# wangjunchi/LLMSeg

Measured on AMD Instinct MI355X. Metric: images/sec (1024x1024, 64-tok prompt) model_forward fwd+bwd, higher is better.
Workload: dtype bf16; 1 GPU; BASELINE.json configs[2]: synthetic 1024x1024 + random-init LLaVA-7B(Llama-7B+CLIP-L/14)/SAM-ViT-H, batch_size=2 per GPU, fwd+bwd train step (CE + align + IoP losses, LoRA r=8 dropout 0.05 on q/v + trainable embed/lm_head/text_fcs/lisa_*, frozen towers, fp32 gradient arena, AdamW step every 10 micro-steps inside the timed region, micro-step replayed from a hipGraph), 256 candidate masks, 64-token ; global_batch=2, parallelism=dp1, graph=True, valid=True

## Files before the change

llmseg_amd/csrc/capi.cpp:

```cpp
#include <hip/hip_runtime.h>
#include <stdarg.h>
#include <stdio.h>
#include <stdlib.h>
#include <algorithm>
#include <array>
#include <map>
#include <mutex>
#include <string>
#include <vector>
#include "llmseg_hip.h"

static thread_local char g_err[512] = "";

void llmseg_set_error(const char* fmt, ...) {
  va_list ap;
  va_start(ap, fmt);
  vsnprintf(g_err, sizeof(g_err), fmt, ap);
  va_end(ap);
}

extern "C" const char* llmseg_last_error(void) { return g_err; }

#include <atomic>
static std::atomic<long> g_launches{0};
// ... 73 lines not shown
    float t = 0;
    (void)hipEventElapsedTime(&t, r.a, r.b);
    ms += t;
    fl += r.flops;
    auto& c = by_class[((r.tag[3] % 10000) / 1000) * 2 + (r.tag[3] & 1)];
    c[0] += t; c[1] += r.flops; c[2] += 1;
    {
      const long S = r.tag[3] / 10000;
      auto& sp = split_by_class[((r.tag[3] % 10000) / 1000) * 2 + (r.tag[3] & 1)];
      if (S > 1) { sp[0] += 1; sp[1] += S; }
    }
    c[3] += 2.0 * ((double)r.tag[0] * r.tag[2] + (double)r.tag[1] * r.tag[2] + (double)r.tag[0] * r.tag[1]);
    auto& e = by_shape[{r.tag[0], r.tag[1], r.tag[2], r.tag[3]}];
    e[0] += t; e[1] += r.flops; e[2] += 1;
    g_pool.push_back(r);
  }
  if (getenv("LLMSEG_PROF_TABLE")) {
    std::vector<std::pair<double, std::array<long, 4>>> order;
    for (auto& kv : by_shape) order.push_back({-kv.second[0], kv.first});
    std::sort(order.begin(), order.end());
    fprintf(stderr, "%8s %8s %8s %6s %8s %10s %9s %6s\n", "M", "N", "K", "var", "calls", "total_ms", "TFLOP/s", "%time");
    const size_t top = (size_t)std::max(40, atoi(getenv("LLMSEG_PROF_TABLE")));
    for (size_t i = 0; i < order.size() && i < top; ++i) {
      auto& e = by_shape[order[i].second];
      fprintf(stderr, "%8ld %8ld %8ld %6ld %8.0f %10.2f %9.1f %6.1f\n", order[i].second[0], order[i].second[1], order[i].second[2], order[i].second[3],
              e[2], e[0], e[1] / (e[0] * 1e-3) / 1e12, 100.0 * e[0] / ms);
    }
  }
  if (total_ms) *total_ms = ms;
  if (total_flops) *total_flops = fl;
  if (launches) *launches = (int64_t)g_recs.size();
  long dom = -1;
  for (auto& kv : by_class) if (dom < 0 || kv.second[0] > by_class[dom][0]) dom = kv.first;
  static const char* names[] = {"gemm_bf16_tn_kernel<*, ...> (register staging, 128x128)", "?", "gemm_bf16_tn_glds_kernel<*, 2, 1>", "gemm_skinny_kernel<M>", "?", "?", "gemm_bf16_tn_t160_kernel (K-sliced)", "gemm_bf16_tn_pp2_kernel<*, false>",
                                "gemm_bf16_tn_pp_kernel<*, false, 4>", "gemm_bf16_tn_pp_kernel<*, false, 2>"};
  if (dom >= 0) {
    const long v = dom / 2;
    std::string nm = (v >= 0 && v < 10) ? names[v] : "?";
    const size_t star = nm.find('*');
    if (star != std::string::npos) nm.replace(star, 1, (dom & 1) ? "true" : "false");
    snprintf(g_dom_name, sizeof(g_dom_name), "%s", nm.c_str());
  } else g_dom_name[0] = 0;
  if (dom_ms) *dom_ms = dom >= 0 ? by_class[dom][0] : 0;
  if (dom_flops) *dom_flops = dom >= 0 ? by_class[dom][1] : 0;
  if (dom_launches) *dom_launches = dom >= 0 ? (int64_t)by_class[dom][2] : 0;
  g_dom_bytes = dom >= 0 ? by_class[dom][3] : 0;
  if (dom >= 0) {
    const auto& sp = split_by_class[dom];
    g_dom_info[0] = (int64_t)by_class[dom][2]; g_dom_info[1] = sp[0]; g_dom_info[2] = sp[1]; g_dom_info[3] = (int64_t)by_class[dom][2] + sp[0];
  } else g_dom_info[0] = g_dom_info[1] = g_dom_info[2] = g_dom_info[3] = 0;
  g_recs.clear();
  return LLMSEG_OK;
}
```

llmseg_amd/csrc/gemm.hip:

```cpp
#include <algorithm>
#include <cstdlib>
#include "common.h"
#include "llmseg_hip.h"

namespace {

constexpr int BN = 128, BK = 64, NT = 256;
constexpr int GROUP_M = 8;

struct GemmP {
  const bf16_t* A; const bf16_t* W; void* C;
  const bf16_t* bias; const bf16_t* gamma; const bf16_t* res;
  int M, N, K;
  long lda, ldw, ldc, ldr, sA, sW, sC, sA2, sW2, sC2;
  int batch1;
  float alpha;
  int act;
  int tiles_m, tiles_n;
  int c_vec, r_vec, b_vec;
  const bf16_t* A2; const bf16_t* W2; long lda2, ldw2;
  int group_m;
  int skew;
  int kt_total;
  int accum;
// ... 890 lines not shown
  const int n = n0 + wn * 64 + c * 4;
  const int mw = m0 + wm * 80;
  float* cbase = reinterpret_cast<float*>(p.C) + b1 * p.sC;
#pragma unroll
  for (int i = 0; i < 3; ++i) {
    const int nh = i < 2 ? 2 : 1;
#pragma unroll
    for (int h = 0; h < nh; ++h)
#pragma unroll
      for (int nb = 0; nb < 4; ++nb) {
        const int row = h * 16 + r15, chunk = nb * 4 + q4;
        *reinterpret_cast<float4*>(slab + row * 64 + ((chunk ^ (row & 15)) << 2)) =
            make_float4(acc[nb][2 * i + h][0], acc[nb][2 * i + h][1], acc[nb][2 * i + h][2], acc[nb][2 * i + h][3]);
      }
#pragma unroll
    for (int it = 0; it < 4 * nh; ++it) {
      const int row = it * 4 + rsub;
      const float4 a4 = *reinterpret_cast<const float4*>(slab + row * 64 + ((c ^ (row & 15)) << 2));
      const int m = mw + i * 32 + row;
      if (m >= p.M || n >= p.N) continue;
      *reinterpret_cast<float4*>(cbase + (long)m * p.ldc + n) =
          make_float4(fmaf(a4.x, p.alpha, 0.f), fmaf(a4.y, p.alpha, 0.f), fmaf(a4.z, p.alpha, 0.f), fmaf(a4.w, p.alpha, 0.f));
    }
  }
}
#undef T160_BL
#undef T160_ISSUE_A0
#undef T160_ISSUE_A1
#undef T160_ISSUE_W
#undef T160_VM_TILE
#undef T160_READ_A
#undef T160_MMA

template <int MT, int AT, bool SK = false>
__global__ __launch_bounds__(256) void gemm_skinny_kernel(GemmP p, int out_f32) {
  constexpr int KS = MT >= 4 ? 1 : 2;
  constexpr int STEP = KS * 512;
  constexpr int ADV = SK ? 4 * STEP : STEP;
  constexpr int XB = AT == 2 ? MT : 1;
  const int lane = threadIdx.x & 63, wave = threadIdx.x >> 6;
  const int n0 = SK ? blockIdx.x * 4 : (blockIdx.x * 4 + wave) * 4;
  if (n0 >= p.N) return;
  const bf16_t* wr[4];
#pragma unroll
  for (int r = 0; r < 4; ++r) wr[r] = p.W + (long)min(n0 + r, p.N - 1) * p.ldw;
  float acc[4][MT];
#pragma unroll
  for (int r = 0; r < 4; ++r)
#pragma unroll
    for (int m = 0; m < MT; ++m) acc[r][m] = 0.f;
  const int K = p.K;
  auto loadw = [&](uint4 (&w)[KS][4], int k) {
#pragma unroll
    for (int t = 0; t < KS; ++t)
#pragma unroll
      for (int r = 0; r < 4; ++r) w[t][r] = *reinterpret_cast<const uint4*>(wr[r] + min(k + t * 512, K - 8));
  };
  auto loadx = [&](uint4 (&xa)[KS][MT], uint4 (&xb)[KS][XB], int k) {
#pragma unroll
    for (int t = 0; t < KS; ++t) {
      const int kk = k + t * 512, kc = min(kk, K - 8);
      const bool ok = kk < K;
#pragma unroll
      for (int m = 0; m < MT; ++m) {
        const bf16_t* ar = p.A + (long)min(m, p.M - 1) * p.lda;
        const uint4 v = *reinterpret_cast<const uint4*>(ar + kc);
// ... 239 lines not shown
    const int c = threadIdx.x + 256 * i;
    if (c < nch) {
      const int n = c * 8;
      const float* sp = slab + m * p.N + n;
      float4 a0 = *reinterpret_cast<const float4*>(sp), a1 = *reinterpret_cast<const float4*>(sp + 4);
      for (int s2 = 1; s2 < S; ++s2) {
        const float4 b0 = *reinterpret_cast<const float4*>(sp + s2 * slab_sz), b1 = *reinterpret_cast<const float4*>(sp + s2 * slab_sz + 4);
        a0.x += b0.x; a0.y += b0.y; a0.z += b0.z; a0.w += b0.w;
        a1.x += b1.x; a1.y += b1.y; a1.z += b1.z; a1.w += b1.w;
      }
      const float v[8] = {a0.x * p.alpha, a0.y * p.alpha, a0.z * p.alpha, a0.w * p.alpha, a1.x * p.alpha, a1.y * p.alpha, a1.z * p.alpha, a1.w * p.alpha};
      const uint4 g = pack8(v);
      *reinterpret_cast<uint4*>(reinterpret_cast<bf16_t*>(p.C) + m * p.ldc + n) = g;
      float of[8], df[8];
      unpack8(*reinterpret_cast<const uint4*>(O + m * ldo + n), of);
      unpack8(g, df);
      float part = 0.f;
#pragma unroll
      for (int e = 0; e < 8; ++e) part = fmaf(of[e], df[e], part);
#pragma unroll
      for (int mm = 8; mm >= 1; mm >>= 1) part += __shfl_xor(part, mm, 64);
      if ((c & 15) == 0) delta[(b * heads + (c >> 4)) * T + q] = part;
    }
  }
}

enum GemmKernel {
  K_REG = 0,
  K_GLDS = 2,
  K_AUTO = 5,
  K_PP256 = 8,
  K_PP128 = 9,
  K_T160 = 10,
};
inline bool is_pp(GemmKernel k) { return k == K_PP256 || k == K_PP128 || k == K_T160; }
inline int pp_rows(GemmKernel k) { return k == K_PP256 ? 256 : k == K_T160 ? T160_BM : 128; }
inline GemmKernel kernel_of_knob(int v) { return v == K_REG || v == K_GLDS || is_pp((GemmKernel)v) ? (GemmKernel)v : K_AUTO; }

template <bool OUT_F32, bool EXT, int FX = FX_NONE>
void launch_pp(GemmKernel k, const GemmP& p, dim3 grid, hipStream_t s) {
  if (k == K_PP256) LL_LAUNCH_KERNEL((gemm_bf16_tn_pp_kernel<OUT_F32, EXT, FX>), grid, dim3(NTB), 0, s, p);
  else LL_LAUNCH_KERNEL((gemm_bf16_tn_pp2_kernel<OUT_F32, EXT, FX>), grid, dim3(NTB), 0, s, p);
}

enum TailKind {
  TAIL_NORM,
  TAIL_NB,
  TAIL_DL,
  TAIL_FX,
};
struct GemmTail { TailKind kind; const llmseg_gemm_args* req; bool done; };

}

void llmseg_prof_begin(hipStream_t s);
void llmseg_prof_end(hipStream_t s, double flops);
void llmseg_prof_tag(long a, long b, long c, long d);

static int g_gemm_variant = K_AUTO, g_gemm_skew = 13, g_gemm_split = 0;
static const bool g_gemm_t160 = getenv("LLMSEG_GEMM_NO_T160") == nullptr;
static const int g_gemm_rsplit = getenv("LLMSEG_GEMM_NO_RSPLIT") ? 0 : 1;
static int num_cus() {
  static int n = [] { int dev = 0, v = 0; (void)hipGetDevice(&dev); (void)hipDeviceGetAttribute(&v, hipDeviceAttributeMultiprocessorCount, dev); return v > 0 ? v : 256; }();
  return n;
}
extern "C" int llmseg_gemm_set_variant(int v) {
  g_gemm_variant = v & 15;
  if ((v >> 4) & 15) g_gemm_skew = ((v >> 4) & 15) - 1;
  g_gemm_split = (v >> 8) & 31;
  return LLMSEG_OK;
}

namespace {
struct GemmPlan { GemmKernel kernel; int split; double us; };
constexpr double T160_KT_US = 1.13;
inline double pp_cost(long M, long N, int nt, int bm, int S, long ncu, bool f32out) {
  const long tiles = ((M + bm - 1) / bm) * ((N + 255) / 256);
  const long rounds = (tiles * S + ncu - 1) / ncu;
  const int q = (nt + S - 1) / S;
  const double it = bm == 256 ? 1.7 : bm == 160 ? T160_KT_US : 1.0, fix = (bm == 256 ? 7.0 : 4.5) + ((S > 1 || f32out) ? 1.0 : 0.0);
  double eff_rounds = (double)rounds;
  if (S == 1) {
    const long full = tiles / ncu, rem = tiles - full * ncu;
    eff_rounds = (double)full + (rem ? 0.5 + 0.5 * (double)rem / (double)ncu : 0.0);
  }
  double us = eff_rounds * (q * it + fix);
  if (S > 1) us += 2.5 + ((double)(S + 1) * M * N * 4.0) / 4.0e6;
  return us;
}
inline double glds_cost(long M, long N, int nt, long ncu) {
  const long tiles = ((M + 127) / 128) * ((N + 127) / 128);
  const long full = tiles / (4 * ncu), rem = tiles - full * 4 * ncu;
  double us = (double)full * (nt * 2.4 + 4.0);
  if (rem > 0) { const double w = (double)((rem + ncu - 1) / ncu); us += nt * std::max(1.3, 0.6 * w) + 4.0; }
  return us;
}
inline bool split_ok(int nt, int S) {
  if (S <= 1) return S == 1;
  const int q = (nt + S - 1) / S;
  return q >= 2 && nt - (S - 1) * q >= 2;
}
}

static int gemm_dispatch(const llmseg_gemm_args* a, void* stream, GemmTail* tail);

extern "C" int llmseg_norm(const void* x, const void* w, const void* b, void* y, int64_t rows, int64_t cols, int64_t ldx, int64_t ldy, float eps, int rms,
                           const int32_t* row_map, void* stream);

extern "C" int llmseg_rope(void* x, const float* cos, const float* sin, int64_t rows, int64_t T, int32_t heads, int32_t head_dim, int64_t ld, void* stream);
extern "C" int llmseg_swiglu(const void* gu, void* out, int64_t rows, int64_t I, int64_t ldgu, int64_t ldo, void* stream);
extern "C" __attribute__((visibility("hidden"))) int llmseg_swiglu_bwd_ld(const void* gu, const void* dout, void* dgu, int64_t rows, int64_t I, int64_t ld_dout, void* stream);

static const bool g_fx_off = getenv("LLMSEG_GEMM_NO_FX") != nullptr;
// ... 107 lines not shown
  LL_CHECK((a->lda & 7) == 0 && (a->ldw & 7) == 0, "gemm: lda/ldw must be multiples of 8 (lda=%ld ldw=%ld)", (long)a->lda, (long)a->ldw);
  const long k8 = (a->K + 7) & ~7L;
  LL_CHECK((ta || (a->K & 7) == 0 || a->lda >= k8) && (tw || (a->K & 7) == 0 || a->ldw >= k8),
           "gemm: K=%ld is not a multiple of 8 and the K-contiguous operand is not padded", (long)a->K);
  LL_CHECK((!ta || a->lda >= a->M) && (!tw || a->ldw >= a->N), "gemm: transposed operand needs ld >= rows");
  LL_CHECK((((uintptr_t)a->A) & 15) == 0 && (((uintptr_t)a->W) & 15) == 0, "gemm: A/W must be 16-byte aligned");
  LL_CHECK(((a->strideA | a->strideW | a->strideA2 | a->strideW2) & 7) == 0, "gemm: batch strides of A/W must be multiples of 8");
  LL_CHECK(!a->accumulate || a->out_f32, "gemm: accumulate needs fp32 output");
  const int esz = a->out_f32 ? 4 : 2;
  GemmP p;
  p.A = (const bf16_t*)a->A; p.W = (const bf16_t*)a->W; p.C = a->C;
  p.bias = (const bf16_t*)a->bias; p.gamma = (const bf16_t*)a->gamma; p.res = (const bf16_t*)a->residual;
  p.M = (int)a->M; p.N = (int)a->N; p.K = (int)a->K;
  p.lda = a->lda; p.ldw = a->ldw; p.ldc = a->ldc; p.ldr = a->residual ? a->ldr : 0;
  const long batch1 = a->batch > 0 ? a->batch : 1, batch2 = a->batch2 > 0 ? a->batch2 : 1;
  const long batch = batch1 * batch2;
  p.batch1 = (int)batch1;
  p.sA = a->strideA; p.sW = a->strideW; p.sC = a->strideC;
  p.sA2 = a->strideA2; p.sW2 = a->strideW2; p.sC2 = a->strideC2;
  p.alpha = a->alpha; p.act = a->act;
  p.kt_total = 0; p.k_split_total = 0; p.accum = a->accumulate ? 1 : 0;
  p.fx = 0; p.fx_T = a->fx_T; p.fx_cols = (int)a->fx_cols; p.fx_I = a->fx == LLMSEG_FX_SWIGLU ? (int)(a->N / 2) : (int)a->N;
  p.fx_cos = a->fx_cos; p.fx_sin = a->fx_sin; p.fx_out = (bf16_t*)a->fx_out; p.fx_in = (const bf16_t*)a->fx_in; p.fx_ld = a->fx_ld;
  p.c_vec = ((((uintptr_t)a->C) % (4 * esz)) == 0 && (a->ldc & 3) == 0 && ((a->strideC | a->strideC2) & 3) == 0) ? 1 : 0;
  p.r_vec = (p.res && (((uintptr_t)p.res) & 7) == 0 && (p.ldr & 3) == 0 && ((a->strideC | a->strideC2) & 3) == 0) ? 1 : 0;
  p.b_vec = ((p.bias == nullptr || (((uintptr_t)p.bias) & 7) == 0) && (p.gamma == nullptr || (((uintptr_t)p.gamma) & 7) == 0)) ? 1 : 0;

  p.skew = g_gemm_skew;
  p.A2 = (const bf16_t*)a->A2; p.W2 = (const bf16_t*)a->W2; p.lda2 = a->lda2; p.ldw2 = a->ldw2;
  static const int group_m_env = getenv("LLMSEG_GEMM_GROUP_M") ? atoi(getenv("LLMSEG_GEMM_GROUP_M")) : 0;
  const int nt = p.K / BK;
  const long ncu = num_cus();
  GemmKernel kernel = (p.K % BK == 0 && !ta && !tw) ? kernel_of_knob(g_gemm_variant) : K_REG;
  if ((kernel == K_PP256 || kernel == K_PP128) && nt < (a->A2 ? 1 : 2)) kernel = K_GLDS;
  if (kernel == K_T160 && nt < 2) kernel = K_GLDS;
  const bool can_split = batch == 1 && (p.N & 3) == 0 && (p.ldc & 3) == 0 && a->workspace != nullptr &&
                         (((uintptr_t)a->workspace) & 15) == 0 && (!p.res || (p.ldr & 3) == 0);
  auto ws_fits = [&](int S) { return (double)(S + (a->A2 ? 1 : 0)) * p.M * p.N * 4.0 <= (double)a->workspace_bytes; };
  int split = 1;
  if (kernel == K_AUTO) {
    GemmPlan best{K_GLDS, 1, glds_cost(p.M, p.N, nt, ncu) * (double)batch};
    if (nt >= (a->A2 ? 1 : 2)) {
      const bool t160 = g_gemm_t160 && !a->fx && !a->residual;
      for (const GemmKernel k : {K_PP256, K_PP128, K_T160}) {
        if (k == K_T160 && !t160) continue;
        const int bm = pp_rows(k);
        for (int S = k == K_T160 ? 2 : 1; S <= 16; ++S) {
          if (S > 1 && (!can_split || !split_ok(nt, S) || !ws_fits(S))) continue;
          if (S > 1 && ((p.M + bm - 1) / bm) * ((p.N + 255) / 256) * S > ncu) break;
          const double us = pp_cost(p.M, p.N, nt, bm, S, ncu, a->out_f32 != 0) * (double)batch;
          if (us < best.us * 0.97 || (us < best.us && S == 1)) best = GemmPlan{k, S, us};
        }
      }
    }
    kernel = best.kernel; split = best.split;
  } else if (kernel == K_PP256 || kernel == K_PP128) {
    split = g_gemm_split > 1 ? g_gemm_split : 1;
    if (split > 1) LL_CHECK(can_split && split_ok(nt, split) && ws_fits(split), "gemm: forced split-K %d not possible for this call", split);
  } else if (kernel == K_T160) {
    split = g_gemm_split;
    LL_CHECK(split > 1 && can_split && split_ok(nt, split) && ws_fits(split), "gemm: variant 10 (160 x 256, K-sliced) needs a forced split-K count >= 2 that is possible for this call (got %d)", split);
  }
  if (p.A2) {
    LL_CHECK(p.W2 && batch == 1 && !ta && !tw && (p.lda2 & 7) == 0 && (p.ldw2 & 7) == 0 && p.lda2 >= 64 && p.ldw2 >= 64 &&
                 (((uintptr_t)p.A2 | (uintptr_t)p.W2) & 15) == 0, "gemm: bad extension operands (A2 [M][64], W2 [N][64], 16-byte aligned rows)");
    LL_CHECK(!a->out_f32, "gemm: extension operands need bf16 output");
    if (is_pp(kernel) && split > 1) {
      llmseg_gemm_args g2 = *a;
      g2.A = a->A2; g2.W = a->W2; g2.lda = a->lda2; g2.ldw = a->ldw2; g2.K = 64; g2.A2 = g2.W2 = nullptr;
      g2.bias = g2.gamma = g2.residual = nullptr; g2.alpha = 1.f; g2.act = LLMSEG_ACT_NONE; g2.out_f32 = 1; g2.accumulate = 0;
      g2.C = (float*)a->workspace + (long)split * p.M * p.N; g2.ldc = p.N; g2.workspace = nullptr; g2.workspace_bytes = 0;
      const int rc = gemm_dispatch(&g2, stream, nullptr);
      if (rc != LLMSEG_OK) return rc;
    } else if (!is_pp(kernel)) {
      LL_CHECK(a->act == LLMSEG_ACT_NONE && !a->gamma, "gemm: extension operands on this shape need a linear epilogue");
      llmseg_gemm_args g1 = *a, g2 = *a;
      g1.A2 = g1.W2 = nullptr;
      int rc = gemm_dispatch(&g1, stream, nullptr);
      if (rc != LLMSEG_OK) return rc;
      g2.A = a->A2; g2.W = a->W2; g2.lda = a->lda2; g2.ldw = a->ldw2; g2.K = 64; g2.bias = nullptr; g2.residual = a->C; g2.ldr = a->ldc;
      g2.A2 = g2.W2 = nullptr;
      return gemm_dispatch(&g2, stream, nullptr);
    }
  }
  p.a_norm_w = (const bf16_t*)a->a_norm_w; p.a_norm_eps = a->a_norm_eps; p.a_swiglu = a->a_swiglu;
  const bool a_xform = p.a_norm_w || p.a_swiglu;
  LL_CHECK(!a_xform || (p.M <= 8 && !ta && !tw && batch == 1 && !p.A2 && (p.K & 7) == 0 && !(p.a_norm_w && p.a_swiglu) &&
                        (!p.a_norm_w || (((uintptr_t)p.a_norm_w) & 15) == 0) && (!p.a_swiglu || p.lda >= 2 * p.K)),
           "gemm: A-row transforms (a_norm_w / a_swiglu) are decode-step fusions of the M <= 8 route");
  if (p.M <= 8 && !ta && !tw && batch == 1 && !p.A2 && (p.K & 7) == 0 && (g_gemm_variant == K_AUTO || a_xform)) {
    hipStream_t s = (hipStream_t)stream;
    llmseg_prof_begin(s);
    llmseg_prof_tag(p.M, p.N, p.K, 3000 + (p.res ? 20 : 0) + p.act * 2 + (a->out_f32 ? 1 : 0));
    static const int sk_env = getenv("LLMSEG_SKINNY_SK") ? atoi(getenv("LLMSEG_SKINNY_SK")) : 1;
    const bool sk = sk_env == 2 ? p.K >= 2048 : (sk_env && p.N <= 8192 && p.K >= 2048);
    const dim3 grid((unsigned)(sk ? (p.N + 3) / 4 : (p.N + 15) / 16));
    const int of = a->out_f32 ? 1 : 0;
#define LL_SKINNY_(AT, SKV)                                                                                   \
    do {                                                                                                      \
      if (p.M == 1) LL_LAUNCH_KERNEL((gemm_skinny_kernel<1, AT, SKV>), grid, dim3(256), 0, s, p, of);      \
      else if (p.M == 2) LL_LAUNCH_KERNEL((gemm_skinny_kernel<2, AT, SKV>), grid, dim3(256), 0, s, p, of); \
      else if (p.M <= 4) LL_LAUNCH_KERNEL((gemm_skinny_kernel<4, AT, SKV>), grid, dim3(256), 0, s, p, of); \
      else LL_LAUNCH_KERNEL((gemm_skinny_kernel<8, AT, SKV>), grid, dim3(256), 0, s, p, of);               \
    } while (0)
#define LL_SKINNY(AT) do { if (sk) LL_SKINNY_(AT, true); else LL_SKINNY_(AT, false); } while (0)
    if (p.a_norm_w) LL_SKINNY(1); else if (p.a_swiglu) LL_SKINNY(2); else LL_SKINNY(0);
#undef LL_SKINNY_
#undef LL_SKINNY
    llmseg_prof_end(s, 2.0 * (double)a->M * (double)a->N * (double)a->K);
    LL_LAUNCH_CHECK("gemm_skinny");
    return LLMSEG_OK;
  }
  const bool pp = is_pp(kernel);
  const int bm = pp ? pp_rows(kernel) : 128, bn = pp ? 256 : BN;
  p.tiles_m = (p.M + bm - 1) / bm; p.tiles_n = (p.N + bn - 1) / bn;
  p.group_m = group_m_env > 0 ? group_m_env : (p.tiles_m <= 32 ? ((p.tiles_n > 16 && p.tiles_m > 8) ? 8 : p.tiles_m) : 4);
  hipStream_t s = (hipStream_t)stream;
  llmseg_prof_begin(s);
  llmseg_prof_tag(p.M, p.N, p.K, (kernel == K_PP128 ? 7 : kernel == K_T160 ? 6 : (int)kernel) * 1000 + (ta ? 200 : 0) + (tw ? 100 : 0) + (p.res ? 20 : 0) + p.act * 2 + (a->out_f32 ? 1 : 0) + 40 * (batch > 1) +
                  10000 * (split > 1 ? split : 0));
  const bool f = a->out_f32 != 0;
  if (kernel == K_REG && batch2 == 1 && (p.N & 3) == 0 && (p.ldc & 3) == 0 && a->workspace != nullptr && (((uintptr_t)a->workspace) & 15) == 0 &&
      (!p.res || ((p.ldr & 3) == 0 && batch == 1)) && ((p.sC & 3) == 0 || batch == 1) && g_gemm_rsplit) {
    const long tiles = (long)p.tiles_m * p.tiles_n * batch;
    const int ntr = (p.K + BK - 1) / BK;
    int S = (tiles * 4 <= ncu && ntr >= 8) ? (int)std::min<long>({(long)ncu / std::max<long>(tiles, 1), (long)ntr / 2, 32L}) : 1;
    while (S > 1 && (double)S * batch * p.M * p.N * 4.0 > (double)a->workspace_bytes) --S;
    if (S > 1) {
      const int q = (ntr + S - 1) / S;
      S = (ntr + q - 1) / q;
    }
    if (S > 1) {
      const int q = (ntr + S - 1) / S;
      GemmP ps = p;
      ps.K = q * BK; ps.k_split_total = p.K; ps.batch1 = S;
      ps.sA = ta ? (long)q * BK * p.lda : (long)q * BK; ps.sW = tw ? (long)q * BK * p.ldw : (long)q * BK;
      ps.sA2 = p.sA; ps.sW2 = p.sW;
      ps.C = a->workspace; ps.ldc = p.N; ps.sC = (long)p.M * p.N; ps.sC2 = (long)S * p.M * p.N;
      ps.bias = ps.gamma = ps.res = nullptr; ps.ldr = 0; ps.alpha = 1.f; ps.act = LLMSEG_ACT_NONE; ps.accum = 0;
      ps.c_vec = 1; ps.r_vec = 0; ps.b_vec = 1;
      const dim3 grid(p.tiles_m * p.tiles_n, (unsigned)(S * batch));
      const int key = (ta ? 2 : 0) | (tw ? 1 : 0);
      switch (key) {
        case 0: LL_LAUNCH_KERNEL((gemm_bf16_tn_kernel<true, false, false>), grid, dim3(NT), 0, s, ps); break;
        case 1: LL_LAUNCH_KERNEL((gemm_bf16_tn_kernel<true, false, true>), grid, dim3(NT), 0, s, ps); break;
        case 2: LL_LAUNCH_KERNEL((gemm_bf16_tn_kernel<true, true, false>), grid, dim3(NT), 0, s, ps); break;
        default: LL_LAUNCH_KERNEL((gemm_bf16_tn_kernel<true, true, true>), grid, dim3(NT), 0, s, ps); break;
      }
      const long total4 = (long)p.M * (p.N >> 2);
      const unsigned rg = (unsigned)std::min<long>((total4 + 255) / 256, 4096);
      LL_LAUNCH_KERNEL(splitk_reduce_kernel, dim3(rg, (unsigned)batch), dim3(256), 0, s, p, (const float*)a->workspace, S, f ? 1 : 0);
      llmseg_prof_end(s, 2.0 * (double)a->M * (double)a->N * (double)a->K * (double)batch);
// ... 16 lines not shown
    const int S2 = split + (p.A2 ? 1 : 0);
    const int cpt = ((p.N >> 3) + 255) / 256;
    const llmseg_gemm_args* r = tail ? tail->req : nullptr;
    static const long wg_max_rows = getenv("LLMSEG_NORM_WG_MAX") ? atol(getenv("LLMSEG_NORM_WG_MAX")) : 2048;
    const bool fuse_norm = tail && tail->kind == TAIL_NORM && !f && p.alpha == 1.f && !p.bias && !p.gamma && p.act == LLMSEG_ACT_NONE && p.M >= 64 && p.M < wg_max_rows &&
                           p.N >= 2048 && p.N <= 8192 && (p.N & 7) == 0 && (p.ldc & 7) == 0 && (!p.res || (p.ldr & 7) == 0) && (r->ldn & 7) == 0 &&
                           ((((uintptr_t)p.C) | ((uintptr_t)p.res) | ((uintptr_t)r->norm_w) | ((uintptr_t)r->norm_out)) & 15) == 0;
    const bool fuse_nb = tail && tail->kind == TAIL_NB && !f && p.alpha == 1.f && !p.bias && !p.gamma && !p.res && p.act == LLMSEG_ACT_NONE && p.M >= 64 && p.N >= 2048 &&
                         p.N <= 8192 && (p.N & 7) == 0;
    const bool fuse_dl = tail && tail->kind == TAIL_DL && !f && !p.bias && !p.gamma && !p.res && p.act == LLMSEG_ACT_NONE && p.N <= 8192 && (p.N & 127) == 0 && (p.ldc & 7) == 0;
    if (fuse_dl) {
#define LL_RDL(C) LL_LAUNCH_KERNEL(splitk_reduce_delta_kernel<C>, dim3((unsigned)p.M), dim3(256), 0, s, p, slabs, S2, (const bf16_t*)r->dl_o, (long)r->dl_ldo, r->dl_out, \
                                   (int)r->dl_heads, (int)r->dl_T)
      if (cpt <= 1) LL_RDL(1); else if (cpt <= 2) LL_RDL(2); else LL_RDL(4);
#undef LL_RDL
    } else if (fuse_nb) {
      const int rc = llmseg_reduce_lora_normbwd(slabs, S2, p.M, p.N, r->nb_x, r->nb_w, r->C, r->nb_eps, r->nb_rms, r->nb_dres, (void*)r->nb_lora_t, r->nb_lora_ldt, r->nb_lora_w0,
                                                r->nb_lora_w1, r->nb_lora_alpha, (const llmseg_dropout*)r->nb_lora_drop, r->nb_lora_part, r->nb_lora_S, r->nb_lora_scale,
                                                r->nb_lora_zero, stream);
      if (rc != LLMSEG_OK) return rc;
    } else if (fuse_norm) {
#define LL_RNORM(C) LL_LAUNCH_KERNEL(splitk_reduce_rmsnorm_kernel<C>, dim3((unsigned)p.M), dim3(256), 0, s, p, slabs, S2, (const bf16_t*)r->norm_w, r->norm_eps, \
                                     (bf16_t*)r->norm_out, (long)r->ldn)
      if (cpt <= 1) LL_RNORM(1); else if (cpt <= 2) LL_RNORM(2); else LL_RNORM(4);
#undef LL_RNORM
    } else {
      const long total4 = (long)p.M * (p.N >> 2);
      const unsigned rg = (unsigned)std::min<long>((total4 + 255) / 256, 4096);
      LL_LAUNCH_KERNEL(splitk_reduce_kernel, dim3(rg), dim3(256), 0, s, p, slabs, S2, f ? 1 : 0);
    }
    if (fuse_dl || fuse_nb || fuse_norm) tail->done = true;
  } else if (pp) {
    dim3 grid(p.tiles_m * p.tiles_n, (unsigned)batch);
    const bool fx_ok = tail && tail->kind == TAIL_FX && !f && batch == 1 &&
                       (a->fx == LLMSEG_FX_ROPE ? (p.N % 256) == 0 && p.A2 != nullptr
                        : a->fx == LLMSEG_FX_SWIGLU ? (p.fx_I % 128) == 0 : (p.N % 64) == 0);
    if (fx_ok) {
      GemmP q = p;
      q.fx = a->fx;
      if (a->fx == LLMSEG_FX_SWIGLU_BWD) q.C = (bf16_t*)a->C - a->N;
      if (a->fx == LLMSEG_FX_ROPE) launch_pp<false, true, FX_ROPE>(kernel, q, grid, s);
      else if (a->fx == LLMSEG_FX_SWIGLU) launch_pp<false, false, FX_SWIGLU>(kernel, q, grid, s);
      else launch_pp<false, false, FX_SWIGLU_BWD>(kernel, q, grid, s);
      tail->done = true;
    } else if (p.A2) launch_pp<false, true>(kernel, p, grid, s);
    else if (f) launch_pp<true, false>(kernel, p, grid, s);
    else launch_pp<false, false>(kernel, p, grid, s);
  } else {
    dim3 grid(p.tiles_m * p.tiles_n, (unsigned)batch);
    if (kernel == K_GLDS) {
      if (f) LL_LAUNCH_KERNEL((gemm_bf16_tn_glds_kernel<true>), grid, dim3(NT), 0, s, p);
      else LL_LAUNCH_KERNEL((gemm_bf16_tn_glds_kernel<false>), grid, dim3(NT), 0, s, p);
    } else {
      const int key = (f ? 4 : 0) | (ta ? 2 : 0) | (tw ? 1 : 0);
      switch (key) {
        case 0: LL_LAUNCH_KERNEL((gemm_bf16_tn_kernel<false, false, false>), grid, dim3(NT), 0, s, p); break;
        case 1: LL_LAUNCH_KERNEL((gemm_bf16_tn_kernel<false, false, true>), grid, dim3(NT), 0, s, p); break;
        case 2: LL_LAUNCH_KERNEL((gemm_bf16_tn_kernel<false, true, false>), grid, dim3(NT), 0, s, p); break;
        case 3: LL_LAUNCH_KERNEL((gemm_bf16_tn_kernel<false, true, true>), grid, dim3(NT), 0, s, p); break;
        case 4: LL_LAUNCH_KERNEL((gemm_bf16_tn_kernel<true, false, false>), grid, dim3(NT), 0, s, p); break;
        case 5: LL_LAUNCH_KERNEL((gemm_bf16_tn_kernel<true, false, true>), grid, dim3(NT), 0, s, p); break;
        case 6: LL_LAUNCH_KERNEL((gemm_bf16_tn_kernel<true, true, false>), grid, dim3(NT), 0, s, p); break;
        default: LL_LAUNCH_KERNEL((gemm_bf16_tn_kernel<true, true, true>), grid, dim3(NT), 0, s, p); break;
      }
    }
  }
// ... 5 lines not shown
```

Measured before the change: 51.35 images/s.

## Add 256x160 tile GEMM kernel and select it via cost model

Adds a new buffer-load-to-LDS pipelined GEMM kernel using 256x160 output tiles with triple buffering and a split epilogue (64+16 column parts). The planner now considers this tile when N is a multiple of 160 and there is no fused extra operand or effect, using its own per-k-tile and fixed cost constants. The aim is to cut tile quantisation waste and improve CU fill for GEMMs whose N does not divide evenly into 256-wide tiles. It adds considerable kernel complexity, and the cost-model constants could pick it in cases where it runs slower.

```diff
diff --git a/llmseg_amd/csrc/capi.cpp b/llmseg_amd/csrc/capi.cpp
--- a/llmseg_amd/csrc/capi.cpp
+++ b/llmseg_amd/csrc/capi.cpp
@@ -129,7 +129,7 @@
   if (launches) *launches = (int64_t)g_recs.size();
   long dom = -1;
   for (auto& kv : by_class) if (dom < 0 || kv.second[0] > by_class[dom][0]) dom = kv.first;
-  static const char* names[] = {"gemm_bf16_tn_kernel<*, ...> (register staging, 128x128)", "?", "gemm_bf16_tn_glds_kernel<*, 2, 1>", "gemm_skinny_kernel<M>", "?", "?", "gemm_bf16_tn_t160_kernel (K-sliced)", "gemm_bf16_tn_pp2_kernel<*, false>",
+  static const char* names[] = {"gemm_bf16_tn_kernel<*, ...> (register staging, 128x128)", "?", "gemm_bf16_tn_glds_kernel<*, 2, 1>", "gemm_skinny_kernel<M>", "gemm_bf16_tn_n160_kernel<*>", "?", "gemm_bf16_tn_t160_kernel (K-sliced)", "gemm_bf16_tn_pp2_kernel<*, false>",
                                 "gemm_bf16_tn_pp_kernel<*, false, 4>", "gemm_bf16_tn_pp_kernel<*, false, 2>"};
   if (dom >= 0) {
     const long v = dom / 2;
diff --git a/llmseg_amd/csrc/gemm.hip b/llmseg_amd/csrc/gemm.hip
--- a/llmseg_amd/csrc/gemm.hip
+++ b/llmseg_amd/csrc/gemm.hip
@@ -946,6 +946,298 @@
 #undef T160_READ_A
 #undef T160_MMA
 
+constexpr int N160_BN = 160;
+#define N160_BL(rs, dst, voff, tt) __builtin_amdgcn_raw_ptr_buffer_load_lds(rs, (lds_ptr_t)(dst), 16, voff, (int)((tt) * (BK * 2)), 0, 0)
+#define N160_ISSUE_A(h, tt, base)                                     \
+  do {                                                                \
+    N160_BL(rsrc_a, (base) + a_lds[h][0], a_off[h][0], tt);           \
+    N160_BL(rsrc_a, (base) + a_lds[h][1], a_off[h][1], tt);           \
+  } while (0)
+#define N160_ISSUE_W0(tt, base) N160_BL(rsrc_w, (base) + w_lds0, w_off0, tt)
+#define N160_ISSUE_W1(tt, base)                                       \
+  do {                                                                \
+    N160_BL(rsrc_w, (base) + w_lds1[0], w_off1[0], tt);               \
+    if (two) N160_BL(rsrc_w, (base) + w_lds1[1], w_off1[1], tt);      \
+  } while (0)
+#define N160_VM_TILE do { if (two) PP_VMI(7); else PP_VMI(6); } while (0)
+#define N160_READ_A(base)                                                                                                     \
+  _Pragma("unroll") for (int mb = 0; mb < 4; ++mb) _Pragma("unroll") for (int ks = 0; ks < 2; ++ks)                         \
+      af[mb][ks] = *reinterpret_cast<const bf16x8_t*>((base) + lds_off(wm * 64 + mb * 16 + frow, ks * 4 + fq))
+#define N160_READ_W(cnt, nb0, base)                                                                                           \
+  _Pragma("unroll") for (int nb = 0; nb < (cnt); ++nb) _Pragma("unroll") for (int ks = 0; ks < 2; ++ks)                     \
+      wf[nb][ks] = *reinterpret_cast<const bf16x8_t*>((base) + A_BYTES + lds_off(wn * 80 + ((nb0) + nb) * 16 + frow, ks * 4 + fq))
+#define N160_MMA(cnt, nb0)                                                                                                    \
+  _Pragma("unroll") for (int ks = 0; ks < 2; ++ks) _Pragma("unroll") for (int nb = 0; nb < (cnt); ++nb)                     \
+      _Pragma("unroll") for (int mb = 0; mb < 4; ++mb)                                                                        \
+          acc[(nb0) + nb][mb] = __builtin_amdgcn_mfma_f32_16x16x32_bf16(wf[nb][ks], af[mb][ks], acc[(nb0) + nb][mb], 0, 0, 0)
+
+template <int LPR>
+struct N160Part {
+  static constexpr int NB = LPR / 4, RPI = 64 / LPR, NIT = 32 / RPI, RS = 4 * LPR;
+  static __device__ __forceinline__ int off(int row, int chunk) { return row * RS + ((chunk ^ (LPR == 16 ? (row & 15) : ((row >> 2) & 3))) << 2); }
+  static __device__ __forceinline__ void stage(float* slab, const f32x4_t (&acc)[5][4], int nb0, int lane, int i) {
+    const int r15 = lane & 15, q = lane >> 4;
+#pragma unroll
+    for (int h = 0; h < 2; ++h)
+#pragma unroll
+      for (int nb = 0; nb < NB; ++nb) {
+        const f32x4_t v = acc[nb0 + nb][2 * i + h];
+        *reinterpret_cast<float4*>(slab + off(h * 16 + r15, nb * 4 + q)) = make_float4(v[0], v[1], v[2], v[3]);
+      }
+  }
+};
+
+template <bool OUT_F32, int ACT, int LPR>
+__device__ __forceinline__ void epilogue_n160_body(const GemmP& p, const f32x4_t (&acc)[5][4], float* slab, int mw, int nc, int nb0, int lane, long bz) {
+  using P = N160Part<LPR>;
+  const int c = lane & (LPR - 1), rsub = lane / LPR;
+  const int n = nc + c * 4;
+  float bs[4] = {0.f, 0.f, 0.f, 0.f}, gm[4] = {1.f, 1.f, 1.f, 1.f};
+  if (p.bias) ld4bf(p.bias + n, true, 4, bs);
+  if (p.gamma) ld4bf(p.gamma + n, true, 4, gm);
+  const long row0 = (long)(mw + rsub);
+  char* cp = reinterpret_cast<char*>(p.C) + (bz + row0 * p.ldc + n) * (OUT_F32 ? 4 : 2);
+  const long cstep = P::RPI * p.ldc * (OUT_F32 ? 4 : 2);
+  const bf16_t* rp = p.res ? p.res + bz + row0 * p.ldr + n : nullptr;
+  const long rstep = P::RPI * p.ldr;
+  const float alpha = p.alpha;
+  const bool has_gamma = p.gamma != nullptr;
+  const bool accum = OUT_F32 && p.accum != 0;
+#pragma unroll
+  for (int i = 0; i < 2; ++i) {
+    uint2 rpre[P::NIT];
+    if (rp) {
+#pragma unroll
+      for (int it = 0; it < P::NIT; ++it) { rpre[it] = *reinterpret_cast<const uint2*>(rp); rp += rstep; }
+    }
+    P::stage(slab, acc, nb0, lane, i);
+#pragma unroll
+    for (int it = 0; it < P::NIT; ++it) {
+      const float4 a4 = *reinterpret_cast<const float4*>(slab + P::off(it * P::RPI + rsub, c));
+      float v[4] = {fmaf(a4.x, alpha, bs[0]), fmaf(a4.y, alpha, bs[1]), fmaf(a4.z, alpha, bs[2]), fmaf(a4.w, alpha, bs[3])};
+      if (ACT == LLMSEG_ACT_GELU) {
+        const f32x2_t g0 = gelu2(f32x2_t{v[0], v[1]}), g1 = gelu2(f32x2_t{v[2], v[3]});
+        v[0] = g0.x; v[1] = g0.y; v[2] = g1.x; v[3] = g1.y;
+      } else if (ACT != LLMSEG_ACT_NONE) {
+#pragma unroll
+        for (int e = 0; e < 4; ++e) v[e] = apply_act(v[e], ACT);
+      }
+      if (has_gamma) {
+#pragma unroll
+        for (int e = 0; e < 4; ++e) v[e] *= gm[e];
+      }
+      if (rp) {
+        v[0] += __uint_as_float(rpre[it].x << 16); v[1] += __uint_as_float(rpre[it].x & 0xffff0000u);
+        v[2] += __uint_as_float(rpre[it].y << 16); v[3] += __uint_as_float(rpre[it].y & 0xffff0000u);
+      }
+      if (OUT_F32) {
+        if (accum) {
+          const float4 o4 = *reinterpret_cast<const float4*>(cp);
+          v[0] += o4.x; v[1] += o4.y; v[2] += o4.z; v[3] += o4.w;
+        }
+        *reinterpret_cast<float4*>(cp) = make_float4(v[0], v[1], v[2], v[3]);
+      } else *reinterpret_cast<uint2*>(cp) = make_uint2(pack2bf(v[0], v[1]), pack2bf(v[2], v[3]));
+      cp += cstep;
+    }
+  }
+}
+
+template <bool OUT_F32, int LPR>
+__device__ __forceinline__ void epilogue_n160_edge(const GemmP& p, const f32x4_t (&acc)[5][4], float* slab, int mw, int nc, int nb0, int lane, long bz) {
+  using P = N160Part<LPR>;
+  const int c = lane & (LPR - 1), rsub = lane / LPR;
+  const int n = nc + c * 4;
+  const int nv = min(4, p.N - n);
+  const bool vec_ok = p.c_vec != 0, res_vec = p.r_vec != 0, b_vec = p.b_vec != 0;
+  const bool fast_cols = vec_ok && b_vec && (!p.res || res_vec) && (n & ~63) + 64 <= p.N;
+  float bs[4] = {0.f, 0.f, 0.f, 0.f}, gm[4] = {1.f, 1.f, 1.f, 1.f};
+  if (nv > 0) {
+    if (p.bias) ld4bf(p.bias + n, b_vec, nv, bs);
+    if (p.gamma) ld4bf(p.gamma + n, b_vec, nv, gm);
+  }
+#pragma unroll
+  for (int i = 0; i < 2; ++i) {
+    const bool fast = fast_cols && ((mw + i * 32) & ~127) + 128 <= p.M;
+    uint2 rpre[P::NIT];
+    if (p.res && res_vec && nv == 4) {
+#pragma unroll
+      for (int it = 0; it < P::NIT; ++it) {
+        const int m = min(mw + i * 32 + it * P::RPI + rsub, p.M - 1);
+        rpre[it] = *reinterpret_cast<const uint2*>(p.res + bz + (long)m * p.ldr + n);
+      }
+    }
+    P::stage(slab, acc, nb0, lane, i);
+#pragma unroll
+    for (int it = 0; it < P::NIT; ++it) {
+      const int row = it * P::RPI + rsub;
+      const float4 a4 = *reinterpret_cast<const float4*>(slab + P::off(row, c));
+      const int m = mw + i * 32 + row;
+      if (m >= p.M || nv <= 0) continue;
+      float v[4];
+      if (fast) { v[0] = fmaf(a4.x, p.alpha, bs[0]); v[1] = fmaf(a4.y, p.alpha, bs[1]); v[2] = fmaf(a4.z, p.alpha, bs[2]); v[3] = fmaf(a4.w, p.alpha, bs[3]); }
+      else { v[0] = a4.x * p.alpha + bs[0]; v[1] = a4.y * p.alpha + bs[1]; v[2] = a4.z * p.alpha + bs[2]; v[3] = a4.w * p.alpha + bs[3]; }
+      if (fast && p.act == LLMSEG_ACT_GELU) {
+        const f32x2_t g0 = gelu2(f32x2_t{v[0], v[1]}), g1 = gelu2(f32x2_t{v[2], v[3]});
+        v[0] = g0.x; v[1] = g0.y; v[2] = g1.x; v[3] = g1.y;
+      } else if (p.act != LLMSEG_ACT_NONE) {
+#pragma unroll
+        for (int e = 0; e < 4; ++e) v[e] = apply_act(v[e], p.act);
+      }
+      if (p.gamma) {
+#pragma unroll
+        for (int e = 0; e < 4; ++e) v[e] *= gm[e];
+      }
+      if (p.res) {
+        if (res_vec && nv == 4) {
+          v[0] += __uint_as_float(rpre[it].x << 16); v[1] += __uint_as_float(rpre[it].x & 0xffff0000u);
+          v[2] += __uint_as_float(rpre[it].y << 16); v[3] += __uint_as_float(rpre[it].y & 0xffff0000u);
+        } else {
+          float rr[4];
+          ld4bf(p.res + bz + (long)m * p.ldr + n, false, nv, rr);
+#pragma unroll
+          for (int e = 0; e < 4; ++e) v[e] += rr[e];
+        }
+      }
+      if (OUT_F32) {
+        float* cp = reinterpret_cast<float*>(p.C) + bz + (long)m * p.ldc + n;
+        if (p.accum) {
+#pragma unroll
+          for (int e = 0; e < 4; ++e) if (e < nv) v[e] += cp[e];
+        }
+        if (vec_ok && nv == 4) {
+          *reinterpret_cast<float4*>(cp) = make_float4(v[0], v[1], v[2], v[3]);
+        } else {
+#pragma unroll
+          for (int e = 0; e < 4; ++e) if (e < nv) cp[e] = v[e];
+        }
+      } else {
+        bf16_t* cp = reinterpret_cast<bf16_t*>(p.C) + bz + (long)m * p.ldc + n;
+        if (vec_ok && nv == 4) {
+          *reinterpret_cast<uint2*>(cp) = make_uint2(pack2bf(v[0], v[1]), pack2bf(v[2], v[3]));
+        } else {
+#pragma unroll
+          for (int e = 0; e < 4; ++e) if (e < nv) cp[e] = f2bf(v[e]);
+        }
+      }
+    }
+  }
+}
+
+template <bool OUT_F32, int LPR>
+__device__ __forceinline__ void epilogue_n160(const GemmP& p, const f32x4_t (&acc)[5][4], float* slab, int mw, int nc, int nb0, int lane, long bz) {
+  const bool interior = (mw & ~127) + 128 <= p.M && ((nc + 4 * LPR - 1) & ~63) + 64 <= p.N && p.c_vec && p.b_vec && (!p.res || p.r_vec);
+  if (!interior) {
+    epilogue_n160_edge<OUT_F32, LPR>(p, acc, slab, mw, nc, nb0, lane, bz);
+    return;
+  }
+  switch (p.act) {
+    case LLMSEG_ACT_NONE: epilogue_n160_body<OUT_F32, LLMSEG_ACT_NONE, LPR>(p, acc, slab, mw, nc, nb0, lane, bz); break;
+    case LLMSEG_ACT_GELU: epilogue_n160_body<OUT_F32, LLMSEG_ACT_GELU, LPR>(p, acc, slab, mw, nc, nb0, lane, bz); break;
+    case LLMSEG_ACT_QUICKGELU: epilogue_n160_body<OUT_F32, LLMSEG_ACT_QUICKGELU, LPR>(p, acc, slab, mw, nc, nb0, lane, bz); break;
+    case LLMSEG_ACT_SILU: epilogue_n160_body<OUT_F32, LLMSEG_ACT_SILU, LPR>(p, acc, slab, mw, nc, nb0, lane, bz); break;
+    case LLMSEG_ACT_RELU: epilogue_n160_body<OUT_F32, LLMSEG_ACT_RELU, LPR>(p, acc, slab, mw, nc, nb0, lane, bz); break;
+    default: epilogue_n160_body<OUT_F32, LLMSEG_ACT_SIGMOID, LPR>(p, acc, slab, mw, nc, nb0, lane, bz); break;
+  }
+}
+
+template <bool OUT_F32>
+__global__ __launch_bounds__(NTB, 2) void gemm_bf16_tn_n160_kernel(GemmP p) {
+  constexpr int BMB = 256, BNB = N160_BN;
+  constexpr int A_BYTES = BMB * BK * 2, W_BYTES = BNB * BK * 2, BUF = A_BYTES + W_BYTES;
+  __shared__ __attribute__((aligned(16))) char smem[3 * BUF];
+  int bid = blockIdx.x;
+  const int nwg = p.tiles_m * p.tiles_n;
+  {
+    const int q = nwg >> 3, r = nwg & 7, xcd = bid & 7;
+    const int len = q + (xcd < r ? 1 : 0);
+    const int idx = ((bid >> 3) + xcd * p.skew) % len;
+    bid = (xcd < r ? xcd * (q + 1) : r * (q + 1) + (xcd - r) * q) + idx;
+  }
+  const int per_group = p.group_m * p.tiles_n;
+  const int first_m = (bid / per_group) * p.group_m;
+  const int gsz = min(p.tiles_m - first_m, p.group_m);
+  const int m0 = (first_m + (bid % per_group) % gsz) * BMB;
+  const int n0 = ((bid % per_group) / gsz) * BNB;
+
+  const int tid = threadIdx.x, lane = tid & 63;
+  const int wave = __builtin_amdgcn_readfirstlane(tid >> 6);
+  const int wm = wave & 3, wn = wave >> 2;
+  const bool two = wave < 4;
+  const long b1 = blockIdx.y % p.batch1, b2 = blockIdx.y / p.batch1;
+  const long bz = b1 * p.sC + b2 * p.sC2;
+  const bf16_t* __restrict__ Ag = p.A + b1 * p.sA + b2 * p.sA2;
+  const bf16_t* __restrict__ Wg = p.W + b1 * p.sW + b2 * p.sW2;
+  const __amdgpu_buffer_rsrc_t rsrc_a = __builtin_amdgcn_make_buffer_rsrc(const_cast<bf16_t*>(Ag + (long)m0 * p.lda), 0, 0x7fffffff, 0x00020000);
+  const __amdgpu_buffer_rsrc_t rsrc_w = __builtin_amdgcn_make_buffer_rsrc(const_cast<bf16_t*>(Wg + (long)n0 * p.ldw), 0, 0x7fffffff, 0x00020000);
+  auto a_src = [&](int ra0) { const int ra = ra0 + (lane >> 3); return (int)(((long)min(ra, p.M - 1 - m0) * p.lda + (((lane & 7) ^ ((ra >> 1) & 7)) << 3)) * 2); };
+  auto w_src = [&](int rw0) { const int rw = rw0 + (lane >> 3); return (int)(((long)min(rw, p.N - 1 - n0) * p.ldw + (((lane & 7) ^ ((rw >> 1) & 7)) << 3)) * 2); };
+  int a_off[2][2], a_lds[2][2];
+#pragma unroll
+  for (int h = 0; h < 2; ++h) {
+#pragma unroll
+    for (int i = 0; i < 2; ++i) {
+      const int ra0 = h * 128 + i * 64 + wave * 8;
+      a_lds[h][i] = ra0 * 128;
+      a_off[h][i] = a_src(ra0);
+    }
+  }
+  const int rw_0 = (wave >> 2) * 80 + (wave & 3) * 8;
+  const int j1 = 8 + (wave & 3);
+  const int rw_1[2] = {(wave / 6) * 80 + 32 + (wave % 6) * 8, (j1 / 6) * 80 + 32 + (j1 % 6) * 8};
+  const int w_lds0 = A_BYTES + rw_0 * 128, w_off0 = w_src(rw_0);
+  const int w_lds1[2] = {A_BYTES + rw_1[0] * 128, A_BYTES + rw_1[1] * 128};
+  const int w_off1[2] = {w_src(rw_1[0]), w_src(rw_1[1])};
+  const int nt = p.K / BK;
+
+  f32x4_t acc[5][4];
+#pragma unroll
+  for (int nb = 0; nb < 5; ++nb)
+#pragma unroll
+    for (int mb = 0; mb < 4; ++mb) acc[nb][mb] = f32x4_t{0.f, 0.f, 0.f, 0.f};
+  bf16x8_t af[4][2], wf[3][2];
+  const int frow = lane & 15, fq = lane >> 4;
+
+  char* cur = smem;
+  char* nxt = smem + BUF;
+  char* nn = smem + 2 * BUF;
+  N160_ISSUE_W0(0, cur); N160_ISSUE_A(0, 0, cur); N160_ISSUE_A(1, 0, cur); N160_ISSUE_W1(0, cur);
+  N160_ISSUE_W0(1, nxt); N160_ISSUE_A(0, 1, nxt); N160_ISSUE_A(1, 1, nxt); N160_ISSUE_W1(1, nxt);
+  N160_VM_TILE;
+  __builtin_amdgcn_s_barrier();
+  if (wn == 1) __builtin_amdgcn_s_barrier();
+  __builtin_amdgcn_sched_barrier(0);
+
+#define N160_RD_A N160_READ_A(cur); N160_READ_W(2, 0, cur)
+#define N160_RD_B N160_READ_W(3, 2, cur)
+  int t = 0;
+  for (; t < nt - 2; ++t) {
+    PP_PHASE(N160_RD_A, N160_ISSUE_W0(t + 2, nn); N160_ISSUE_A(0, t + 2, nn), PP_NOP, N160_MMA(2, 0));
+    PP_PHASE(N160_RD_B, N160_ISSUE_A(1, t + 2, nn); N160_ISSUE_W1(t + 2, nn), N160_VM_TILE, N160_MMA(3, 2));
+    char* const tmp = cur; cur = nxt; nxt = nn; nn = tmp;
+  }
+  PP_PHASE(N160_RD_A, PP_NOP, PP_NOP, N160_MMA(2, 0));
+  PP_PHASE(N160_RD_B, PP_NOP, PP_VMI(0), N160_MMA(3, 2));
+  cur = nxt;
+  PP_PHASE(N160_RD_A, PP_NOP, PP_NOP, N160_MMA(2, 0));
+  PP_PHASE(N160_RD_B, PP_NOP, PP_NOP, N160_MMA(3, 2));
+#undef N160_RD_A
+#undef N160_RD_B
+  if (wn == 0) __builtin_amdgcn_s_barrier();
+
+  float* slab = reinterpret_cast<float*>(smem) + wave * (32 * 80);
+  const int mw = m0 + wm * 64, nw = n0 + wn * 80;
+  epilogue_n160<OUT_F32, 16>(p, acc, slab, mw, nw, 0, lane, bz);
+  epilogue_n160<OUT_F32, 4>(p, acc, slab + 32 * 64, mw, nw + 64, 4, lane, bz);
+}
+#undef N160_BL
+#undef N160_ISSUE_A
+#undef N160_ISSUE_W0
+#undef N160_ISSUE_W1
+#undef N160_VM_TILE
+#undef N160_READ_A
+#undef N160_READ_W
+#undef N160_MMA
+
 template <int MT, int AT, bool SK = false>
 __global__ __launch_bounds__(256) void gemm_skinny_kernel(GemmP p, int out_f32) {
   constexpr int KS = MT >= 4 ? 1 : 2;
@@ -1251,9 +1543,11 @@
   K_PP256 = 8,
   K_PP128 = 9,
   K_T160 = 10,
+  K_N160 = 11,
 };
-inline bool is_pp(GemmKernel k) { return k == K_PP256 || k == K_PP128 || k == K_T160; }
-inline int pp_rows(GemmKernel k) { return k == K_PP256 ? 256 : k == K_T160 ? T160_BM : 128; }
+inline bool is_pp(GemmKernel k) { return k == K_PP256 || k == K_PP128 || k == K_T160 || k == K_N160; }
+inline int pp_rows(GemmKernel k) { return k == K_PP256 || k == K_N160 ? 256 : k == K_T160 ? T160_BM : 128; }
+inline int pp_cols(GemmKernel k) { return k == K_N160 ? N160_BN : 256; }
 inline GemmKernel kernel_of_knob(int v) { return v == K_REG || v == K_GLDS || is_pp((GemmKernel)v) ? (GemmKernel)v : K_AUTO; }
 
 template <bool OUT_F32, bool EXT, int FX = FX_NONE>
@@ -1278,6 +1572,7 @@
 
 static int g_gemm_variant = K_AUTO, g_gemm_skew = 13, g_gemm_split = 0;
 static const bool g_gemm_t160 = getenv("LLMSEG_GEMM_NO_T160") == nullptr;
+static const bool g_gemm_n160 = getenv("LLMSEG_GEMM_NO_N160") == nullptr;
 static const int g_gemm_rsplit = getenv("LLMSEG_GEMM_NO_RSPLIT") ? 0 : 1;
 static int num_cus() {
   static int n = [] { int dev = 0, v = 0; (void)hipGetDevice(&dev); (void)hipDeviceGetAttribute(&v, hipDeviceAttributeMultiprocessorCount, dev); return v > 0 ? v : 256; }();
@@ -1293,11 +1588,13 @@
 namespace {
 struct GemmPlan { GemmKernel kernel; int split; double us; };
 constexpr double T160_KT_US = 1.13;
-inline double pp_cost(long M, long N, int nt, int bm, int S, long ncu, bool f32out) {
-  const long tiles = ((M + bm - 1) / bm) * ((N + 255) / 256);
+constexpr double N160_KT_US = 1.19, N160_FIX_US = 6.6;
+inline double pp_cost(long M, long N, int nt, int bm, int bn, int S, long ncu, bool f32out) {
+  const long tiles = ((M + bm - 1) / bm) * ((N + bn - 1) / bn);
   const long rounds = (tiles * S + ncu - 1) / ncu;
   const int q = (nt + S - 1) / S;
-  const double it = bm == 256 ? 1.7 : bm == 160 ? T160_KT_US : 1.0, fix = (bm == 256 ? 7.0 : 4.5) + ((S > 1 || f32out) ? 1.0 : 0.0);
+  const double it = bn == N160_BN ? N160_KT_US : bm == 256 ? 1.7 : bm == 160 ? T160_KT_US : 1.0;
+  const double fix = (bn == N160_BN ? N160_FIX_US : bm == 256 ? 7.0 : 4.5) + ((S > 1 || f32out) ? 1.0 : 0.0);
   double eff_rounds = (double)rounds;
   if (S == 1) {
     const long full = tiles / ncu, rem = tiles - full * ncu;
@@ -1471,7 +1768,9 @@
   const int nt = p.K / BK;
   const long ncu = num_cus();
   GemmKernel kernel = (p.K % BK == 0 && !ta && !tw) ? kernel_of_knob(g_gemm_variant) : K_REG;
+  if (kernel == K_N160 && (a->A2 || a->fx)) kernel = K_PP256;
   if ((kernel == K_PP256 || kernel == K_PP128) && nt < (a->A2 ? 1 : 2)) kernel = K_GLDS;
+  if (kernel == K_N160 && nt < 2) kernel = K_GLDS;
   if (kernel == K_T160 && nt < 2) kernel = K_GLDS;
   const bool can_split = batch == 1 && (p.N & 3) == 0 && (p.ldc & 3) == 0 && a->workspace != nullptr &&
                          (((uintptr_t)a->workspace) & 15) == 0 && (!p.res || (p.ldr & 3) == 0);
@@ -1481,13 +1780,15 @@
     GemmPlan best{K_GLDS, 1, glds_cost(p.M, p.N, nt, ncu) * (double)batch};
     if (nt >= (a->A2 ? 1 : 2)) {
       const bool t160 = g_gemm_t160 && !a->fx && !a->residual;
-      for (const GemmKernel k : {K_PP256, K_PP128, K_T160}) {
+      const bool n160 = g_gemm_n160 && !a->fx && !a->A2 && nt >= 2 && p.N % N160_BN == 0;
+      for (const GemmKernel k : {K_PP256, K_PP128, K_T160, K_N160}) {
         if (k == K_T160 && !t160) continue;
-        const int bm = pp_rows(k);
-        for (int S = k == K_T160 ? 2 : 1; S <= 16; ++S) {
+        if (k == K_N160 && (!n160 || best.split > 1)) continue;
+        const int bm = pp_rows(k), bn = pp_cols(k);
+        for (int S = k == K_T160 ? 2 : 1; S <= (k == K_N160 ? 1 : 16); ++S) {
           if (S > 1 && (!can_split || !split_ok(nt, S) || !ws_fits(S))) continue;
           if (S > 1 && ((p.M + bm - 1) / bm) * ((p.N + 255) / 256) * S > ncu) break;
-          const double us = pp_cost(p.M, p.N, nt, bm, S, ncu, a->out_f32 != 0) * (double)batch;
+          const double us = pp_cost(p.M, p.N, nt, bm, bn, S, ncu, a->out_f32 != 0) * (double)batch;
           if (us < best.us * 0.97 || (us < best.us && S == 1)) best = GemmPlan{k, S, us};
         }
       }
@@ -1551,12 +1852,12 @@
     return LLMSEG_OK;
   }
   const bool pp = is_pp(kernel);
-  const int bm = pp ? pp_rows(kernel) : 128, bn = pp ? 256 : BN;
+  const int bm = pp ? pp_rows(kernel) : 128, bn = pp ? pp_cols(kernel) : BN;
   p.tiles_m = (p.M + bm - 1) / bm; p.tiles_n = (p.N + bn - 1) / bn;
-  p.group_m = group_m_env > 0 ? group_m_env : (p.tiles_m <= 32 ? ((p.tiles_n > 16 && p.tiles_m > 8) ? 8 : p.tiles_m) : 4);
+  p.group_m = group_m_env > 0 ? group_m_env : kernel == K_N160 ? 4 : (p.tiles_m <= 32 ? ((p.tiles_n > 16 && p.tiles_m > 8) ? 8 : p.tiles_m) : 4);
   hipStream_t s = (hipStream_t)stream;
   llmseg_prof_begin(s);
-  llmseg_prof_tag(p.M, p.N, p.K, (kernel == K_PP128 ? 7 : kernel == K_T160 ? 6 : (int)kernel) * 1000 + (ta ? 200 : 0) + (tw ? 100 : 0) + (p.res ? 20 : 0) + p.act * 2 + (a->out_f32 ? 1 : 0) + 40 * (batch > 1) +
+  llmseg_prof_tag(p.M, p.N, p.K, (kernel == K_PP128 ? 7 : kernel == K_T160 ? 6 : kernel == K_N160 ? 4 : (int)kernel) * 1000 + (ta ? 200 : 0) + (tw ? 100 : 0) + (p.res ? 20 : 0) + p.act * 2 + (a->out_f32 ? 1 : 0) + 40 * (batch > 1) +
                   10000 * (split > 1 ? split : 0));
   const bool f = a->out_f32 != 0;
   if (kernel == K_REG && batch2 == 1 && (p.N & 3) == 0 && (p.ldc & 3) == 0 && a->workspace != nullptr && (((uintptr_t)a->workspace) & 15) == 0 &&
@@ -1639,6 +1940,13 @@
     if (fuse_dl || fuse_nb || fuse_norm) tail->done = true;
   } else if (pp) {
     dim3 grid(p.tiles_m * p.tiles_n, (unsigned)batch);
+    if (kernel == K_N160) {
+      if (f) LL_LAUNCH_KERNEL((gemm_bf16_tn_n160_kernel<true>), grid, dim3(NTB), 0, s, p);
+      else LL_LAUNCH_KERNEL((gemm_bf16_tn_n160_kernel<false>), grid, dim3(NTB), 0, s, p);
+      llmseg_prof_end(s, 2.0 * (double)a->M * (double)a->N * (double)a->K * (double)batch);
+      LL_LAUNCH_CHECK("gemm_bf16_tn (256 x 160)");
+      return LLMSEG_OK;
+    }
     const bool fx_ok = tail && tail->kind == TAIL_FX && !f && batch == 1 &&
                        (a->fx == LLMSEG_FX_ROPE ? (p.N % 256) == 0 && p.A2 != nullptr
                         : a->fx == LLMSEG_FX_SWIGLU ? (p.fx_I % 128) == 0 : (p.N % 64) == 0);
```

Result: no change. 50.99 images/s (-0.7%).
